# JeffreyXiang/ivid

Hardware: NVIDIA H100
Metric: 128x128 RGBD multiview samples/sec (higher is better)
Workload: dtype fp16 tensor-core operands, fp32 accumulate / residual stream / GroupNorm / softmax / sampler

## Files before the change

ivid_b200/csrc/conv_gemm.cuh:

```cuda
#pragma once
#include <type_traits>

#include "common.cuh"

namespace ivid {

struct ConvGemmParams {
  int N, H, W;
  int TW, TH, TN;
  int tiles_w, tiles_h, tiles_n;
  int n_blocks;
  int seg_chunks[3];
  int seg_taps[3];
  int Cout;
  int ldc;
  int ldr;
  int out_mode;
  const float* bias;
  const float* residual;
  int res_up;
  void* out;
  __half* out16;
  double* stats;
  float acc_scale;
};

struct ConvMaps {
  CUtensorMap a[3];
  CUtensorMap b;
};
struct ConvMaps8 : ConvMaps {
  CUtensorMap b8;
};

template <int BN>
struct ConvGemmCfg {
  static constexpr int BM = 128;
  static constexpr int BK = 64;
  static constexpr int A_BYTES = BM * BK * 2;
  static constexpr int B_BYTES = ((BN * BK * 2 + 1023) / 1024) * 1024;
  static constexpr int STAGE_BYTES = A_BYTES + B_BYTES;
  static constexpr int STAGES = BN == 128 ? 3 : 4;
  static constexpr int BAR_BYTES = 128;
  static constexpr int STAT_BYTES = 8 * 2 * BN * 4;
  static constexpr int SMEM_BYTES = STAGES * STAGE_BYTES + BAR_BYTES + STAT_BYTES + 1024;
  static constexpr int CONSUMER_THREADS = 256;
  static constexpr int THREADS = CONSUMER_THREADS + 32;
};

struct ConvKCursor {
  int seg = 0, t = 0, ch = 0, base = 0;
};

template <int BN, bool A8 = false>
__global__ void __launch_bounds__(ConvGemmCfg<BN>::THREADS, 2)
conv_gemm_kernel(const __grid_constant__ std::conditional_t<A8, ConvMaps8, ConvMaps> maps, const __grid_constant__ ConvGemmParams p) {
  using Cfg = ConvGemmCfg<BN>;
  constexpr int STAGES = Cfg::STAGES;
  extern __shared__ uint8_t smem_raw[];
  uint8_t* smem = smem_raw + ((1024u - (smem_u32(smem_raw) & 1023u)) & 1023u);
  uint64_t* full_bar = reinterpret_cast<uint64_t*>(smem + STAGES * Cfg::STAGE_BYTES);
  uint64_t* empty_bar = full_bar + STAGES;
  float* stat_smem = reinterpret_cast<float*>(smem + STAGES * Cfg::STAGE_BYTES + Cfg::BAR_BYTES);

  const int tid = threadIdx.x;
  const int warp = tid >> 5, lane = tid & 31;
  const int wg = warp >> 2;

  if (tid == 0) {
    for (int s = 0; s < STAGES; ++s) {
      mbar_init(&full_bar[s], 1);
      mbar_init(&empty_bar[s], 8u);
    }
    fence_barrier_init();
  }
  __syncthreads();

  int nunits = 0;
  for (int sg = 0; sg < 3; ++sg) nunits += p.seg_chunks[sg] * p.seg_taps[sg];
  const int nunits8 = A8 ? p.seg_chunks[0] * p.seg_taps[0] : 0;

  const int mt = static_cast<int>(blockIdx.x) / p.n_blocks, nb = static_cast<int>(blockIdx.x) % p.n_blocks;
  const int colbase = nb * BN;
  const int tiles_per_img = p.tiles_w * p.tiles_h;
  const int tn = mt / tiles_per_img;
  const int rem = mt - tn * tiles_per_img;
  const int th = rem / p.tiles_w;
  const int tw = rem - th * p.tiles_w;
  const int n0 = tn * p.TN, h0 = th * p.TH, w0 = tw * p.TW;

  if (warp == Cfg::CONSUMER_THREADS / 32) {
    if (lane == 0) {
      tma_prefetch_desc(&maps.a[0]);
      tma_prefetch_desc(&maps.b);
      if constexpr (A8) tma_prefetch_desc(&maps.b8);
      ConvKCursor c;
      while (p.seg_chunks[c.seg] == 0) ++c.seg;
#pragma unroll 1
      for (int u = 0; u < nunits; ++u) {
        const uint32_t g = static_cast<uint32_t>(u);
        const int s = static_cast<int>(g % STAGES);
        if (g >= STAGES) mbar_wait(&empty_bar[s], ((g / STAGES) - 1) & 1);
        const int taps = p.seg_taps[c.seg], chunks = p.seg_chunks[c.seg];
        uint8_t* sa = smem + s * Cfg::STAGE_BYTES;
        uint8_t* sb = sa + Cfg::A_BYTES;
        const int dy = (taps == 9) ? (c.t / 3 - 1) : 0;
        const int dx = (taps == 9) ? (c.t % 3 - 1) : 0;
        mbar_arrive_expect_tx(&full_bar[s], Cfg::A_BYTES + BN * Cfg::BK * 2);
        bool e4m3 = false;
        if constexpr (A8) {
          if (c.seg == 0) {
            tma_load_4d(&maps.a[0], &full_bar[s], sa, c.ch * 128, w0 + dx, h0 + dy, n0);
            tma_load_2d(&maps.b8, &full_bar[s], sb, (c.t * chunks + c.ch) * 128, colbase);
            e4m3 = true;
          }
        }
        if (!e4m3) {
          const int kcol = c.base + (c.t * chunks + c.ch) * 64;
          tma_load_4d(&maps.a[c.seg], &full_bar[s], sa, c.ch * 64, w0 + dx, h0 + dy, n0);
          tma_load_2d(&maps.b, &full_bar[s], sb, kcol, colbase);
        }
        if (++c.ch == chunks) {
          c.ch = 0;
          if (++c.t == taps) { c.t = 0; if (!A8 || c.seg != 0) c.base += taps * chunks * 64; ++c.seg; }
        }
        while (c.seg < 3 && p.seg_chunks[c.seg] == 0) ++c.seg;
      }
    }
    return;
  }

  float acc[BN / 2];
#pragma unroll
  for (int i = 0; i < BN / 2; ++i) acc[i] = 0.f;

#pragma unroll 1
  for (int u = 0; u < nunits; ++u) {
    const uint32_t g = static_cast<uint32_t>(u);
    const int s = static_cast<int>(g % STAGES);
    mbar_wait(&full_bar[s], (g / STAGES) & 1);
    const uint32_t sa = smem_u32(smem + s * Cfg::STAGE_BYTES);
    const uint32_t sb = sa + Cfg::A_BYTES;
    wgmma_fence();
    const uint64_t da = make_smem_desc_sw128(sa + wg * 64 * 128, 1024, 16);
    const uint64_t db = make_smem_desc_sw128(sb, 1024, 16);
    if (A8 && u < nunits8) {
#pragma unroll
      for (int k = 0; k < 4; ++k) wgmma_ss_e4m3<BN>(acc, da + 2 * k, db + 2 * k, (u | k) != 0 ? 1u : 0u);
    } else {
#pragma unroll
      for (int k = 0; k < 4; ++k) wgmma_ss<BN>(acc, da + 2 * k, db + 2 * k, (u | k) != 0 ? 1u : 0u);
    }
    wgmma_commit();
    wgmma_wait<1>();
    if (u > 0 && lane == 0) mbar_arrive(&empty_bar[(g - 1) % STAGES]);
  }
  wgmma_wait<0>();
  reg_fence(acc);
  if (lane == 0) mbar_arrive(&empty_bar[static_cast<uint32_t>(nunits - 1) % STAGES]);

  const int wr = warp & 3;
  const int quad = lane & 3;
  uint32_t pix[2], rpix[2];
  bool ok[2];
#pragma unroll
  for (int i = 0; i < 2; ++i) {
    const int row = wg * 64 + wr * 16 + (lane >> 2) + 8 * i;
    const int n = n0 + row / (p.TW * p.TH), h = h0 + (row / p.TW) % p.TH, x = w0 + row % p.TW;
    ok[i] = n < p.N;
    pix[i] = (static_cast<uint32_t>(n) * p.H + h) * p.W + x;
    rpix[i] = p.res_up ? (static_cast<uint32_t>(n) * (p.H >> 1) + (h >> 1)) * (p.W >> 1) + (x >> 1) : pix[i];
  }
  const bool do_stats = p.stats != nullptr;
#pragma unroll
  for (int j = 0; j < BN / 8; ++j) {
    const int c = colbase + 8 * j + 2 * quad;
    float s0 = 0.f, s1 = 0.f, q0 = 0.f, q1 = 0.f;
    if (c < p.Cout) {
      const float2 b = make_float2(__ldg(p.bias + c), __ldg(p.bias + c + 1));
#pragma unroll
      for (int i = 0; i < 2; ++i) {
        if (!ok[i]) continue;
        float v0, v1;
        if (A8) {
          v0 = fmaf(acc[4 * j + 2 * i], p.acc_scale, b.x); v1 = fmaf(acc[4 * j + 2 * i + 1], p.acc_scale, b.y);
        } else {
          v0 = acc[4 * j + 2 * i] + b.x; v1 = acc[4 * j + 2 * i + 1] + b.y;
        }
        if (p.out_mode == 2) {
          const uint32_t hw = static_cast<uint32_t>(p.H) * p.W, n = pix[i] / hw;
          float* o = reinterpret_cast<float*>(p.out) + (static_cast<size_t>(n) * p.Cout + c) * hw + (pix[i] - n * hw);
          o[0] = v0;
          if (c + 1 < p.Cout) o[hw] = v1;
          continue;
        }
        if (p.residual != nullptr) {
          const float2 r = __ldg(reinterpret_cast<const float2*>(p.residual + static_cast<size_t>(rpix[i]) * p.ldr + c));
          v0 += r.x; v1 += r.y;
        }
        if (p.out_mode == 0) {
          *reinterpret_cast<float2*>(reinterpret_cast<float*>(p.out) + static_cast<size_t>(pix[i]) * p.ldc + c) = make_float2(v0, v1);
          if (p.out16 != nullptr) *reinterpret_cast<uint32_t*>(p.out16 + static_cast<size_t>(pix[i]) * p.ldc + c) = pack_h2(v0, v1);
        } else {
          const __half2 hv = __floats2half2_rn(v0, v1);
          *reinterpret_cast<__half2*>(reinterpret_cast<__half*>(p.out) + static_cast<size_t>(pix[i]) * p.ldc + c) = hv;
          const float2 r = __half22float2(hv);
          v0 = r.x; v1 = r.y;
        }
        s0 += v0; s1 += v1;
        q0 = fmaf(v0, v0, q0); q1 = fmaf(v1, v1, q1);
      }
    }
    if (do_stats) {
#pragma unroll
      for (int off = 4; off < 32; off <<= 1) {
        s0 += __shfl_xor_sync(0xffffffffu, s0, off);
        s1 += __shfl_xor_sync(0xffffffffu, s1, off);
        q0 += __shfl_xor_sync(0xffffffffu, q0, off);
        q1 += __shfl_xor_sync(0xffffffffu, q1, off);
      }
      if (lane < 4) {
        float* st = stat_smem + warp * 2 * BN + 8 * j + 2 * quad;
        st[0] = s0; st[1] = s1; st[BN] = q0; st[BN + 1] = q1;
      }
    }
  }
  if (do_stats) {
    asm volatile("bar.sync 1, %0;\n" ::"n"(Cfg::CONSUMER_THREADS) : "memory");
    const int rows_per_n = p.TW * p.TH;
    const int n_tile = (128 + rows_per_n - 1) / rows_per_n;
    for (int e = tid; e < n_tile * BN; e += Cfg::CONSUMER_THREADS) {
      const int sn = e / BN, c = e - sn * BN;
      const int n = n0 + sn, col = colbase + c;
      if (n >= p.N || col >= p.Cout) continue;
      float ssum = 0.f, qsum = 0.f;
      for (int w8 = 0; w8 < 8; ++w8) {
        if ((w8 * 16) / rows_per_n != sn) continue;
        ssum += stat_smem[w8 * 2 * BN + c];
        qsum += stat_smem[w8 * 2 * BN + BN + c];
      }
      double* st = p.stats + (static_cast<size_t>(n) * p.Cout + col) * 2;
      atomicAdd(st, static_cast<double>(ssum));
      atomicAdd(st + 1, static_cast<double>(qsum));
    }
  }
}

}
```

ivid_b200/csrc/ops.cu:

```cuda
#include "ops.h"

#include <algorithm>
#include <cmath>
#include <mutex>

#include "attention.cuh"
#include "attention_hd.cuh"
#include "conv_gemm.cuh"
#include "elementwise.cuh"
#include "embed.cuh"

namespace ivid {

struct ConvLaunch {
  ConvMaps8 maps;
  ConvGemmParams p;
  int BN;
  bool a8;
  int grid;
};

int conv_pad_cout(int cout) {
  if (cout >= 64) return ((cout + 63) / 64) * 64;
  return ((cout + 15) / 16) * 16;
}
static int pow2_divisor(int v, int cap) {
  int t = 1;
  while (t * 2 <= cap && v % (t * 2) == 0) t *= 2;
  return t;
}
void conv_tile(int H, int W, int* TW, int* TH, int* TN) {
  IVID_REQUIRE(H > 0 && W > 0, "conv: spatial size must be positive");
  *TW = pow2_divisor(W, 16);
  *TH = pow2_divisor(H, 128 / *TW);
  *TN = 128 / (*TW * *TH);
}
bool conv_can_fuse_stats(int H, int W) {
  int TW, TH, TN;
  conv_tile(H, W, &TW, &TH, &TN);
  return TW * TH >= 32;
}
int conv_pick_bn(int cout_pad) {
  if (cout_pad % 128 == 0) return 128;
  if (cout_pad % 64 == 0) return 64;
  if (cout_pad % 16 == 0 && cout_pad <= 48) return 16;
  throw Error(kErrInvalidArgument, "conv: unsupported padded Cout " + std::to_string(cout_pad));
}

bool conv_can_res_up(int W, int cout) { return W >= 16 && cout % 8 == 0; }
bool conv_can_out16(int cout) { return cout % 8 == 0; }
int conv_pad_k(int c) { return ((c + 63) / 64) * 64; }
int conv_pad_k8(int c) { return ((c + 127) / 128) * 128; }
int conv_seg_cols(int taps, int c) { return taps * conv_pad_k(c); }

ConvPack conv_pack(const float* w, const float* b, int cout, int cin, int ksz, int pitch, const float* w2, const float* b2,
                   int cin2, int cin2a, bool e4m3) {
  ConvPack pk;
  const int taps = ksz * ksz;
  pk.cout_pad = conv_pad_cout(cout);
  float scale = 1.f;
  if (e4m3) {
    IVID_REQUIRE(pitch == conv_pad_k(cin), "internal: an e4m3 segment 0 is an ordinary 3x3 or 1x1 conv");
    float mx = 0.f;
    for (size_t i = 0; i < static_cast<size_t>(cout) * cin * taps; ++i) mx = std::max(mx, std::fabs(w[i]));
    const int e = fp8_weight_exponent(mx);
    const float kMinNormal16 = std::ldexp(1.0f, -14);
    if (cin % 16 != 0) pk.refused = "its input channels are not a multiple of 16";
    else if (e < -100 || e > 100) pk.refused = "its weight exponent is outside [-100, 100]";
    for (size_t i = 0; pk.refused == nullptr && i < static_cast<size_t>(cout) * cin2; ++i) {
      const float v = std::fabs(w2[i]), sv = v * std::ldexp(1.0f, e);
      if (sv > 65504.f) pk.refused = "its skip weights times 2^e overflow fp16";
      else if (v >= kMinNormal16 && sv < kMinNormal16) pk.refused = "its skip weights times 2^e become fp16 subnormals";
    }
    pk.e4m3 = pk.refused == nullptr;
    if (pk.e4m3) { pk.e = e; scale = std::ldexp(1.0f, e); }
  }
  const int s0 = cin2a > 0 ? cin2a : cin2, s1 = cin2 - s0;
  const int k0 = pk.e4m3 ? 0 : conv_seg_cols(1, taps * pitch);
  pk.K = k0 + conv_seg_cols(1, s0) + conv_seg_cols(1, s1);
  pk.w16.assign(static_cast<size_t>(pk.cout_pad) * pk.K, __float2half_rn(0.f));
  const int cp8 = conv_pad_k8(cin), K8 = pk.e4m3 ? taps * cp8 : 0;
  pk.w8.assign(static_cast<size_t>(pk.cout_pad) * K8, 0);
  for (int co = 0; co < cout; ++co) {
    __half* row = pk.w16.data() + static_cast<size_t>(co) * pk.K;
    for (int tap = 0; tap < taps; ++tap)
      for (int ci = 0; ci < cin; ++ci) {
        const float v = w[(static_cast<size_t>(co) * cin + ci) * taps + tap];
        if (pk.e4m3) pk.w8[static_cast<size_t>(co) * K8 + tap * cp8 + ci] = fp8_e4m3_from_float(v * scale);
        else row[tap * pitch + ci] = __float2half_rn(v);
      }
    for (int ci = 0; ci < cin2; ++ci)
      row[k0 + (ci < s0 ? ci : conv_pad_k(s0) + ci - s0)] = __float2half_rn(w2[static_cast<size_t>(co) * cin2 + ci] * scale);
  }
  pk.bias.assign(pk.cout_pad, 0.f);
  for (int i = 0; i < cout; ++i) {
    if (b != nullptr) pk.bias[i] = b[i];
    if (b2 != nullptr) pk.bias[i] += b2[i];
  }
  return pk;
}

ConvLaunch* conv_launch_create(const ConvDesc& d) {
  IVID_REQUIRE(d.C0 > 0 && d.C0 % 8 == 0, "conv: segment-0 channels must be a positive multiple of 8");
  IVID_REQUIRE(d.C1 % 8 == 0, "conv: segment-1 channels must be a multiple of 8");
  IVID_REQUIRE(d.taps0 == 9 || d.taps0 == 1, "conv: only 3x3 (pad 1) and 1x1 kernels are on this path");
  IVID_REQUIRE(d.taps1 == 9 || d.taps1 == 1, "conv: only 3x3 (pad 1) and 1x1 kernels are on this path");
  IVID_REQUIRE(d.C2 % 8 == 0 && (d.taps2 == 9 || d.taps2 == 1), "conv: segment 2 must be a multiple of 8 channels, 3x3 or 1x1");
  IVID_REQUIRE(d.N > 0 && static_cast<int64_t>(d.N) * d.H * d.W < (int64_t{1} << 31),
               "conv: N*H*W must be below 2^31 (32-bit pixel indices in the epilogue)");
  const bool a8 = d.weight8 != nullptr;
  IVID_REQUIRE(!a8 || d.C0 % 16 == 0, "conv: an e4m3 segment 0 needs a multiple of 16 channels (16-byte TMA rows)");
  auto* l = new ConvLaunch();
  l->a8 = a8;
  ConvGemmParams& p = l->p;
  p.N = d.N; p.H = d.H; p.W = d.W;
  conv_tile(d.H, d.W, &p.TW, &p.TH, &p.TN);
  p.tiles_w = d.W / p.TW;
  p.tiles_h = d.H / p.TH;
  p.tiles_n = (d.N + p.TN - 1) / p.TN;
  l->BN = conv_pick_bn(d.cout_pad);
  p.n_blocks = d.cout_pad / l->BN;
  p.seg_chunks[0] = a8 ? conv_pad_k8(d.C0) / 128 : conv_pad_k(d.C0) / 64; p.seg_taps[0] = d.taps0;
  p.acc_scale = d.acc_scale;
  p.seg_chunks[1] = conv_pad_k(d.C1) / 64; p.seg_taps[1] = d.C1 > 0 ? d.taps1 : 0;
  p.seg_chunks[2] = conv_pad_k(d.C2) / 64; p.seg_taps[2] = d.C2 > 0 ? d.taps2 : 0;
  p.Cout = d.cout; p.ldc = d.ldc; p.ldr = d.ldr; p.out_mode = d.out_mode;
  p.bias = d.bias; p.residual = d.residual; p.out = d.out;
  p.stats = (d.stats != nullptr && conv_can_fuse_stats(d.H, d.W) && d.out_mode != 2) ? d.stats : nullptr;
  IVID_REQUIRE(d.stats == nullptr || p.stats != nullptr, "conv: fused statistics need >= 32 pixels per sample per warp");
  IVID_REQUIRE(d.out_mode == 2 || (d.cout % 8 == 0 && d.ldc % 8 == 0), "conv: NHWC output needs Cout % 8 == 0");
  IVID_REQUIRE(d.residual == nullptr || (d.out_mode != 2 && d.ldr % 2 == 0), "conv: residual needs an NHWC output and an even row pitch");
  p.res_up = 0;
  if (d.residual != nullptr && d.residual_up) {
    IVID_REQUIRE(conv_can_res_up(d.W, d.cout) && d.H % 2 == 0, "conv: upsampled residual needs W >= 16 and Cout % 8 == 0");
    p.res_up = 1;
  }
  p.out16 = nullptr;
  if (d.out16 != nullptr) {
    IVID_REQUIRE(d.out_mode == 0 && conv_can_out16(d.cout), "conv: fp16 output copy needs an fp32 NHWC output and Cout % 8 == 0");
    p.out16 = static_cast<__half*>(d.out16);
  }
  const int Ktot = (a8 ? 0 : conv_seg_cols(d.taps0, d.C0)) + conv_seg_cols(d.taps1, d.C1) + conv_seg_cols(d.taps2, d.C2);
  ConvMaps8& M = l->maps;
  M.a[0] = a8 ? make_act_map(d.act0, d.N, d.H, d.W, d.C0, p.TW, p.TH, p.TN, CU_TENSOR_MAP_DATA_TYPE_UINT8)
              : make_act_map(d.act0, d.N, d.H, d.W, d.C0, p.TW, p.TH, p.TN);
  M.a[1] = d.C1 > 0 ? make_act_map(d.act1, d.N, d.H, d.W, d.C1, p.TW, p.TH, p.TN) : M.a[0];
  M.a[2] = d.C2 > 0 ? make_act_map(d.act2, d.N, d.H, d.W, d.C2, p.TW, p.TH, p.TN) : M.a[0];
  if (a8) {
    M.b8 = make_weight_map(d.weight8, d.cout_pad, d.taps0 * conv_pad_k8(d.C0), l->BN, CU_TENSOR_MAP_DATA_TYPE_UINT8);
    M.b = Ktot > 0 ? make_weight_map(d.weight, d.cout_pad, Ktot, l->BN) : M.b8;
  } else {
    M.b = make_weight_map(d.weight, d.cout_pad, Ktot, l->BN);
  }
  l->grid = p.tiles_w * p.tiles_h * p.tiles_n * p.n_blocks;
  return l;
}
void conv_launch_destroy(ConvLaunch* l) { delete l; }
int conv_launch_bn(const ConvLaunch* l) { return l->BN; }
bool conv_launch_a8(const ConvLaunch* l) { return l->a8; }

template <int BN, bool A8>
static void run_conv(const ConvLaunch* l, cudaStream_t s) {
  using Cfg = ConvGemmCfg<BN>;
  static std::once_flag once;
  std::call_once(once, [] {
    IVID_CHECK_CUDA(cudaFuncSetAttribute(conv_gemm_kernel<BN, A8>, cudaFuncAttributeMaxDynamicSharedMemorySize, Cfg::SMEM_BYTES));
  });
  if constexpr (A8) conv_gemm_kernel<BN, true><<<l->grid, Cfg::THREADS, Cfg::SMEM_BYTES, s>>>(l->maps, l->p);
  else conv_gemm_kernel<BN, false><<<l->grid, Cfg::THREADS, Cfg::SMEM_BYTES, s>>>(static_cast<const ConvMaps&>(l->maps), l->p);
  IVID_CHECK_CUDA(cudaGetLastError());
}
void conv_launch_run_out(const ConvLaunch* l, void* out, cudaStream_t s) {
  ConvLaunch tmp = *l;
  tmp.p.out = out;
  conv_launch_run(&tmp, s);
}
void conv_launch_run(const ConvLaunch* l, cudaStream_t s) {
  if (l->a8) {
    switch (l->BN) {
      case 128: run_conv<128, true>(l, s); break;
      case 64: run_conv<64, true>(l, s); break;
      default: run_conv<16, true>(l, s); break;
    }
    return;
  }
  switch (l->BN) {
    case 128: run_conv<128, false>(l, s); break;
    case 64: run_conv<64, false>(l, s); break;
    default: run_conv<16, false>(l, s); break;
  }
}

struct AttnLaunch {
  CUtensorMap mapQ, mapKV;
  AttnParams p;
  AttnHdParams hp;
  int head_ch = 64;
  int nv = 0;
  bool qres = false;
  int smem = 0;
  int grid;
};

AttnLaunch* attn_launch_create(const void* qkv, int N, int T, int C, int head_ch, void* out) {
  if (head_ch <= 0 || head_ch % 64 != 0)
    throw Error(kErrNotImplemented, "attention: head width " + std::to_string(head_ch) + " is not a multiple of 64");
  IVID_REQUIRE(C % head_ch == 0, "attention: channels must be a multiple of the head width " + std::to_string(head_ch));
  IVID_REQUIRE(T >= 1, "attention: sequence length must be positive");
  auto* l = new AttnLaunch();
  l->head_ch = head_ch;
  l->p.N = N; l->p.T = T; l->p.C = C; l->p.heads = C / 64;
  l->p.q_tiles = (T + 127) / 128;
  l->p.out = reinterpret_cast<__half*>(out);
  const uint64_t dims[3] = {static_cast<uint64_t>(3 * C), static_cast<uint64_t>(T), static_cast<uint64_t>(N)};
  const uint64_t str[2] = {static_cast<uint64_t>(3 * C) * 2, static_cast<uint64_t>(T) * 3 * C * 2};
  const uint32_t boxq[3] = {64, 128, 1};
  const uint32_t boxkv[3] = {64, AttnCfg::KV, 1};
  l->mapQ = make_tensor_map(CU_TENSOR_MAP_DATA_TYPE_FLOAT16, 3, const_cast<void*>(qkv), dims, str, boxq,
                            CU_TENSOR_MAP_SWIZZLE_128B);
  l->mapKV = make_tensor_map(CU_TENSOR_MAP_DATA_TYPE_FLOAT16, 3, const_cast<void*>(qkv), dims, str, boxkv,
                             CU_TENSOR_MAP_SWIZZLE_128B);
  l->grid = N * l->p.heads * l->p.q_tiles;
  if (head_ch == 64) return l;
  using Cfg = AttnHdCfg;
  const int k = head_ch / 64;
  const int slices = (k + 3) / 4;
  l->nv = (k + slices - 1) / slices;
  l->qres = k <= Cfg::RESIDENT_Q_MAX_CHUNKS;
  AttnHdParams& hp = l->hp;
  hp.N = N; hp.T = T; hp.C = C; hp.d = head_ch; hp.heads = C / head_ch; hp.chunks = k;
  hp.q_tiles = l->p.q_tiles;
  hp.slices = (k + l->nv - 1) / l->nv;
  hp.scale_log2 = static_cast<float>(1.4426950408889634 / std::sqrt(static_cast<double>(head_ch)));
  hp.out = l->p.out;
  const int q_bytes = l->qres ? k * Cfg::QCHUNK_BYTES : 0;
  const int fixed = q_bytes + 1024  + 1024 ;
  const int budget = l->nv == 2 ? Cfg::MAX_SMEM_2CTA : Cfg::MAX_SMEM;
  hp.stages = std::min(Cfg::MAX_STAGES, (budget - fixed) / Cfg::stage_bytes(l->qres));
  IVID_REQUIRE(hp.stages >= 4, "attention: shared-memory ring too shallow");
  l->smem = fixed + hp.stages * Cfg::stage_bytes(l->qres);
  l->grid = N * hp.heads * hp.q_tiles * hp.slices;
  return l;
}
void attn_launch_destroy(AttnLaunch* l) { delete l; }

template <int NV, bool QRES>
static void run_attn_hd(const AttnLaunch* l, cudaStream_t s) {
  static std::once_flag once;
  std::call_once(once, [] {
    IVID_CHECK_CUDA(cudaFuncSetAttribute(attention_hd_kernel<NV, QRES>, cudaFuncAttributeMaxDynamicSharedMemorySize, AttnHdCfg::MAX_SMEM));
  });
  attention_hd_kernel<NV, QRES><<<l->grid, AttnHdCfg::THREADS, l->smem, s>>>(l->mapQ, l->mapKV, l->hp);
  IVID_CHECK_CUDA(cudaGetLastError());
}

void attn_launch_run(const AttnLaunch* l, cudaStream_t s) {
  if (l->head_ch != 64) {
    switch (l->nv * 2 + (l->qres ? 1 : 0)) {
      case 5: run_attn_hd<2, true>(l, s); break;
      case 7: run_attn_hd<3, true>(l, s); break;
      case 9: run_attn_hd<4, true>(l, s); break;
      case 4: run_attn_hd<2, false>(l, s); break;
      case 6: run_attn_hd<3, false>(l, s); break;
      case 8: run_attn_hd<4, false>(l, s); break;
      default: throw Error(kErrState, "internal: attention slice width " + std::to_string(l->nv));
    }
    return;
  }
  static std::once_flag once;
  std::call_once(once, [] {
    IVID_CHECK_CUDA(cudaFuncSetAttribute(attention_kernel, cudaFuncAttributeMaxDynamicSharedMemorySize, AttnCfg::SMEM_BYTES));
  });
  attention_kernel<<<l->grid, AttnCfg::THREADS, AttnCfg::SMEM_BYTES, s>>>(l->mapQ, l->mapKV, l->p);
  IVID_CHECK_CUDA(cudaGetLastError());
}

static int ew_grid(size_t work_items, int block) {
  const size_t blocks = (work_items + block - 1) / block;
  const size_t cap = static_cast<size_t>(sm_count()) * 16;
  return static_cast<int>(std::max<size_t>(1, std::min(blocks, cap)));
}

void launch_gn_stats(const float* x, double* stats, int N, int HW, int C, cudaStream_t s) {
  IVID_REQUIRE(C % 4 == 0, "gn_stats: C % 4");
  dim3 grid((HW + kStatsPixPerBlock - 1) / kStatsPixPerBlock, N);
  gn_stats_kernel<<<grid, 256, 0, s>>>(x, stats, HW, C);
  IVID_CHECK_CUDA(cudaGetLastError());
}

void launch_gn_apply(const GnApplyDesc& d, cudaStream_t s) {
  IVID_REQUIRE(d.C0 % 8 == 0 && d.C1 % 8 == 0, "gn_apply: channel counts must be multiples of 8");
  const int C = d.C0 + d.C1;
  IVID_REQUIRE(d.groups >= 1 && d.groups <= 64 && C % d.groups == 0, "group norm: groups must divide channels (<= 64 groups)");
  IVID_REQUIRE(d.stats0 != nullptr && d.gamma != nullptr && d.beta != nullptr, "gn_apply: statistics / affine parameters missing");
  GnApplyParams p;
  p.x0 = static_cast<const float*>(d.x0); p.x1 = static_cast<const float*>(d.x1); p.C0 = d.C0; p.C1 = d.C1; p.N = d.N; p.H = d.H; p.W = d.W; p.mode = d.mode;
  p.x0h = d.x0_half ? reinterpret_cast<const __half*>(d.x0) : nullptr;
  p.x1h = d.x0_half ? reinterpret_cast<const __half*>(d.x1) : nullptr;
  p.silu = d.silu ? 1 : 0;
  p.stats0 = d.stats0; p.stats1 = d.stats1; p.groups = d.groups; p.inv_count = 1.0 / (static_cast<double>(d.H) * d.W);
  p.eps = d.eps; p.gamma = d.gamma; p.beta = d.beta; p.film = d.film; p.film_ld = d.film_ld; p.film_off = d.film_off;
  p.film_add = d.film_add ? 1 : 0;
  p.out_act = reinterpret_cast<__half*>(d.out_act); p.out_raw16 = reinterpret_cast<__half*>(d.out_raw16);
  p.out_act8 = d.out_e4m3 ? reinterpret_cast<uint8_t*>(d.out_act) : nullptr;
  p.out_raw32 = d.out_raw32;
  p.out_lo = reinterpret_cast<__half*>(d.out_lo);
  IVID_REQUIRE(d.out_lo == nullptr || (d.mode == 0 && d.x0_half && d.out_raw16 == nullptr && d.out_raw32 == nullptr),
               "gn_apply: the split (hi/lo) output exists on the same-resolution fp16-source path only");
  IVID_REQUIRE(!d.out_e4m3 || (d.out_lo == nullptr && C % 16 == 0), "gn_apply: an e4m3 output needs C % 16 == 0 and no split output");
  const int Ho = d.mode == 1 ? d.H * 2 : (d.mode == 2 ? d.H / 2 : d.H);
  const int Wo = d.mode == 1 ? d.W * 2 : (d.mode == 2 ? d.W / 2 : d.W);
  {
    const int blocks_per_n = std::max(1, (sm_count() * 3) / std::max(d.N, 1));
    const int by_wave = (Ho * Wo + blocks_per_n - 1) / blocks_per_n;
    const int small = std::max(1, 1024 / (C / 8));
    p.pix_per_block = std::max(1, std::min(Ho * Wo, std::max(by_wave, small)));
  }
  int pix_space = Ho * Wo;
  if (d.mode == 1) {
    pix_space = d.H * d.W;
    p.pix_per_block = std::max(1, (p.pix_per_block + 3) / 4);
  }
  dim3 grid((pix_space + p.pix_per_block - 1) / p.pix_per_block, d.N);
  const size_t smem = static_cast<size_t>(C) * 8;
  if (p.mode == 0 && p.x0h != nullptr && p.out_raw16 == nullptr && p.out_raw32 == nullptr) {
    const bool hoist = 256 % (C / 8) == 0;
    if (p.out_lo != nullptr) {
      if (hoist) gn_apply_h16_kernel<true, true><<<grid, 256, smem, s>>>(p);
      else gn_apply_h16_kernel<false, true><<<grid, 256, smem, s>>>(p);
    } else if (d.out_e4m3) {
      if (hoist) gn_apply_h16_kernel<true, false, true><<<grid, 256, smem, s>>>(p);
      else gn_apply_h16_kernel<false, false, true><<<grid, 256, smem, s>>>(p);
    } else if (hoist) gn_apply_h16_kernel<true><<<grid, 256, smem, s>>>(p);
    else gn_apply_h16_kernel<false><<<grid, 256, smem, s>>>(p);
  } else if (d.out_e4m3) {
    gn_apply_kernel<true><<<grid, 256, smem, s>>>(p);
  } else {
    gn_apply_kernel<><<<grid, 256, smem, s>>>(p);
  }
  IVID_CHECK_CUDA(cudaGetLastError());
}
void launch_im2col_s2(const void* x16, void* col, int N, int H, int W, int C, cudaStream_t s) {
  IVID_REQUIRE(C % 8 == 0 && H % 2 == 0 && W % 2 == 0, "im2col_s2: C % 8, even spatial size");
  const size_t items = static_cast<size_t>(N) * (H / 2) * (W / 2) * 9 * (C / 8);
  im2col_s2_h16_kernel<<<ew_grid(items, 256), 256, 0, s>>>(reinterpret_cast<const __half*>(x16), reinterpret_cast<__half*>(col), N, H, W, C);
  IVID_CHECK_CUDA(cudaGetLastError());
}
void launch_upsample2x_h16(const void* x16, void* out, int N, int H, int W, int C, cudaStream_t s) {
  IVID_REQUIRE(C % 8 == 0, "upsample2x: C % 8");
  const size_t items = static_cast<size_t>(N) * H * W * 4 * (C / 8);
  upsample2x_h16_kernel<<<ew_grid(items, 256), 256, 0, s>>>(reinterpret_cast<const __half*>(x16), reinterpret_cast<__half*>(out), N, H, W, C);
  IVID_CHECK_CUDA(cudaGetLastError());
}
void launch_resample_f32(const float* x, float* out, void* out16, int N, int H, int W, int C, int mode, cudaStream_t s) {
  IVID_REQUIRE(C % 4 == 0 && (mode == 1 || (H % 2 == 0 && W % 2 == 0)), "resample_f32: C % 4, even spatial size for pooling");
  const size_t items = static_cast<size_t>(N) * (mode == 1 ? 4 * H * W : (H / 2) * (W / 2)) * (C / 4);
  resample_f32_kernel<<<ew_grid(items, 256), 256, 0, s>>>(x, out, reinterpret_cast<__half*>(out16), N, H, W, C, mode);
  IVID_CHECK_CUDA(cudaGetLastError());
}
void launch_pack_input(const float* x, void* out, int N, int Nx, int Cin, int HW, cudaStream_t s) {
  IVID_REQUIRE(Cin >= 1 && Cin <= 16, "pack_input: 1..16 input channels (two-term split inside 64 operand channels)");
  pack_input_kernel<<<ew_grid(static_cast<size_t>(N) * HW, 256), 256, 0, s>>>(x, reinterpret_cast<__half*>(out), N, Nx,
                                                                                 Cin, HW);
  IVID_CHECK_CUDA(cudaGetLastError());
}

void launch_eps_gather(const float* Y, const float* bias, float* eps, int N, int H, int W, int Co, int ldy, cudaStream_t s) {
  IVID_REQUIRE(Co >= 1 && Co <= 7 && 9 * Co <= ldy, "eps_gather: 9*Co tap columns must fit the row pitch");
  IVID_REQUIRE(Co != 4 || ldy % 4 == 0, "eps_gather: row pitch must keep float4 alignment");
  eps_gather_kernel<<<ew_grid(static_cast<size_t>(N) * H * W, 256), 256, 0, s>>>(Y, bias, eps, N, H, W, Co, ldy);
  IVID_CHECK_CUDA(cudaGetLastError());
}

void launch_posenc(const int64_t* t, int Nt, const float* freqs, int half, float* out, int N, cudaStream_t s) {
  posenc_kernel<<<N, 128, 0, s>>>(t, Nt, freqs, half, out, N);
  IVID_CHECK_CUDA(cudaGetLastError());
}

void launch_film_table(const float* emb, const float* Wp, const float* bias, float* x_t, float* out, int N, int K, int O, cudaStream_t s) {
  IVID_REQUIRE(K % 32 == 0 && O % 4 == 0, "film table: K % 32 == 0");
  static std::once_flag once;
  std::call_once(once, [] {
    IVID_CHECK_CUDA(cudaFuncSetAttribute(film_table_kernel, cudaFuncAttributeMaxDynamicSharedMemorySize, FilmCfg::SMEM_BYTES));
  });
  const int nblk = (N + 31) / 32;
  silu_transpose_kernel<<<std::min(256, (nblk * K * 32 + 255) / 256), 256, 0, s>>>(emb, x_t, N, K, 1);
  const int tiles = (O + FilmCfg::TO - 1) / FilmCfg::TO;
  dim3 grid(std::min(tiles, std::max(1, sm_count() / nblk)), nblk);
  film_table_kernel<<<grid, FilmCfg::THREADS, FilmCfg::SMEM_BYTES, s>>>(Wp, x_t, bias, out, N, K, O);
  IVID_CHECK_CUDA(cudaGetLastError());
}

void launch_linear(const float* in, const float* W, const float* bias, float* out, int N, int K, int O, int silu_in,
                   const float* label_emb, const int64_t* classes, int Ncls, cudaStream_t s) {
  if ((K == 256 || K == 512 || K == 1024) && O <= 8192) {
    dim3 grid((O + 7) / 8, (N + 31) / 32);
    const size_t smem = static_cast<size_t>(32) * K * 4;
    static std::once_flag once;
    std::call_once(once, [] {
      IVID_CHECK_CUDA(cudaFuncSetAttribute(linear_warp_kernel<2>, cudaFuncAttributeMaxDynamicSharedMemorySize, 32 * 256 * 4));
      IVID_CHECK_CUDA(cudaFuncSetAttribute(linear_warp_kernel<4>, cudaFuncAttributeMaxDynamicSharedMemorySize, 32 * 512 * 4));
      IVID_CHECK_CUDA(cudaFuncSetAttribute(linear_warp_kernel<8>, cudaFuncAttributeMaxDynamicSharedMemorySize, 32 * 1024 * 4));
    });
    auto go = [&](auto kern) { kern<<<grid, 256, smem, s>>>(in, W, bias, out, N, O, silu_in, label_emb, classes, Ncls); };
    if (K == 256) go(linear_warp_kernel<2>); else if (K == 512) go(linear_warp_kernel<4>); else go(linear_warp_kernel<8>);
    IVID_CHECK_CUDA(cudaGetLastError());
    return;
  }
  if (K % 32 == 0) {
    if (O >= 128 * 64) {
      dim3 grid((O + 127) / 128, (N + 31) / 32);
      linear_tiled_kernel<4><<<grid, 256, 0, s>>>(in, W, bias, out, N, K, O, silu_in, label_emb, classes, Ncls);
    } else {
      dim3 grid((O + 63) / 64, (N + 31) / 32);
      linear_tiled_kernel<2><<<grid, 256, 0, s>>>(in, W, bias, out, N, K, O, silu_in, label_emb, classes, Ncls);
    }
    IVID_CHECK_CUDA(cudaGetLastError());
    return;
  }
  dim3 grid((O + 63) / 64, (N + 31) / 32);
  linear_rows_kernel<<<grid, 256, 0, s>>>(in, W, bias, out, N, K, O, silu_in, label_emb, classes, Ncls);
  IVID_CHECK_CUDA(cudaGetLastError());
}

}
```

Measured before the change: 0.3019.

## Reuse a halo activation slab across the three vertical taps in 3x3 convs

For 3x3 convolutions with suitable tiles, the producer loads one taller activation slab (tile height plus two halo rows) per horizontal offset and channel chunk. The three vertical taps then read it by offsetting the wgmma descriptor by whole rows, instead of issuing three separate A loads. A two-slab ring with its own empty barriers is split from the weight ring. This cuts TMA activation traffic roughly threefold for the main segment, at the cost of more complex barrier and slab-index bookkeeping and different shared-memory sizing.

```diff
diff --git a/ivid_b200/csrc/conv_gemm.cuh b/ivid_b200/csrc/conv_gemm.cuh
--- a/ivid_b200/csrc/conv_gemm.cuh
+++ b/ivid_b200/csrc/conv_gemm.cuh
@@ -33,7 +33,7 @@
   CUtensorMap b8;
 };
 
-template <int BN>
+template <int BN, bool SLAB = false>
 struct ConvGemmCfg {
   static constexpr int BM = 128;
   static constexpr int BK = 64;
@@ -41,9 +41,12 @@
   static constexpr int B_BYTES = ((BN * BK * 2 + 1023) / 1024) * 1024;
   static constexpr int STAGE_BYTES = A_BYTES + B_BYTES;
   static constexpr int STAGES = BN == 128 ? 3 : 4;
+  static constexpr int SLAB_BYTES = 160 * 128;
+  static constexpr int SLABS = 2;
+  static constexpr int RING_BYTES = SLAB ? SLABS * SLAB_BYTES + STAGES * B_BYTES : STAGES * STAGE_BYTES;
   static constexpr int BAR_BYTES = 128;
   static constexpr int STAT_BYTES = 8 * 2 * BN * 4;
-  static constexpr int SMEM_BYTES = STAGES * STAGE_BYTES + BAR_BYTES + STAT_BYTES + 1024;
+  static constexpr int SMEM_BYTES = RING_BYTES + BAR_BYTES + STAT_BYTES + 1024;
   static constexpr int CONSUMER_THREADS = 256;
   static constexpr int THREADS = CONSUMER_THREADS + 32;
 };
@@ -52,16 +55,19 @@
   int seg = 0, t = 0, ch = 0, base = 0;
 };
 
-template <int BN, bool A8 = false>
+template <int BN, bool A8 = false, bool SLAB = false>
 __global__ void __launch_bounds__(ConvGemmCfg<BN>::THREADS, 2)
 conv_gemm_kernel(const __grid_constant__ std::conditional_t<A8, ConvMaps8, ConvMaps> maps, const __grid_constant__ ConvGemmParams p) {
-  using Cfg = ConvGemmCfg<BN>;
+  using Cfg = ConvGemmCfg<BN, SLAB>;
   constexpr int STAGES = Cfg::STAGES;
+  constexpr int SLABS = Cfg::SLABS;
   extern __shared__ uint8_t smem_raw[];
   uint8_t* smem = smem_raw + ((1024u - (smem_u32(smem_raw) & 1023u)) & 1023u);
-  uint64_t* full_bar = reinterpret_cast<uint64_t*>(smem + STAGES * Cfg::STAGE_BYTES);
+  uint64_t* full_bar = reinterpret_cast<uint64_t*>(smem + Cfg::RING_BYTES);
   uint64_t* empty_bar = full_bar + STAGES;
-  float* stat_smem = reinterpret_cast<float*>(smem + STAGES * Cfg::STAGE_BYTES + Cfg::BAR_BYTES);
+  uint64_t* slab_empty = empty_bar + STAGES;
+  float* stat_smem = reinterpret_cast<float*>(smem + Cfg::RING_BYTES + Cfg::BAR_BYTES);
+  uint8_t* wring = smem + SLABS * Cfg::SLAB_BYTES;
 
   const int tid = threadIdx.x;
   const int warp = tid >> 5, lane = tid & 31;
@@ -71,6 +77,9 @@
     for (int s = 0; s < STAGES; ++s) {
       mbar_init(&full_bar[s], 1);
       mbar_init(&empty_bar[s], 8u);
+    }
+    if constexpr (SLAB) {
+      for (int s = 0; s < SLABS; ++s) mbar_init(&slab_empty[s], 8u);
     }
     fence_barrier_init();
   }
@@ -89,7 +98,59 @@
   const int tw = rem - th * p.tiles_w;
   const int n0 = tn * p.TN, h0 = th * p.TH, w0 = tw * p.TW;
 
-  if (warp == Cfg::CONSUMER_THREADS / 32) {
+  if (SLAB && warp == Cfg::CONSUMER_THREADS / 32) {
+    if (lane == 0) {
+      tma_prefetch_desc(&maps.a[0]);
+      tma_prefetch_desc(&maps.b);
+      if constexpr (A8) tma_prefetch_desc(&maps.b8);
+      uint32_t u = 0, a = 0;
+      auto issue = [&](const CUtensorMap* am, int ac, int ax, int ay, uint32_t a_bytes, const CUtensorMap* bm, int kcol) {
+        const int s = static_cast<int>(u % STAGES);
+        if (u >= STAGES) mbar_wait(&empty_bar[s], ((u / STAGES) - 1) & 1);
+        const int q = static_cast<int>(a % SLABS);
+        if (a_bytes != 0 && a >= SLABS) mbar_wait(&slab_empty[q], ((a / SLABS) - 1) & 1);
+        mbar_arrive_expect_tx(&full_bar[s], a_bytes + BN * Cfg::BK * 2);
+        if (a_bytes != 0) {
+          tma_load_4d(am, &full_bar[s], smem + q * Cfg::SLAB_BYTES, ac, ax, ay, n0);
+          ++a;
+        }
+        tma_load_2d(bm, &full_bar[s], wring + s * Cfg::B_BYTES, kcol, colbase);
+        ++u;
+      };
+      const int chunks0 = p.seg_chunks[0];
+      const uint32_t slab_bytes = static_cast<uint32_t>(p.TW * (p.TH + 2) * p.TN) * 128u;
+#pragma unroll 1
+      for (int dx = 0; dx < 3; ++dx) {
+#pragma unroll 1
+        for (int ch = 0; ch < chunks0; ++ch) {
+#pragma unroll 1
+          for (int dy = 0; dy < 3; ++dy) {
+            const int t = dy * 3 + dx;
+            const uint32_t ab = dy == 0 ? slab_bytes : 0u;
+            if constexpr (A8) issue(&maps.a[0], ch * 128, w0 + dx - 1, h0 - 1, ab, &maps.b8, (t * chunks0 + ch) * 128);
+            else issue(&maps.a[0], ch * 64, w0 + dx - 1, h0 - 1, ab, &maps.b, (t * chunks0 + ch) * 64);
+          }
+        }
+      }
+      int base = A8 ? 0 : 9 * chunks0 * 64;
+#pragma unroll 1
+      for (int sg = 1; sg < 3; ++sg) {
+        const int taps = p.seg_taps[sg], chunks = p.seg_chunks[sg];
+        if (chunks == 0) continue;
+#pragma unroll 1
+        for (int t = 0; t < taps; ++t) {
+          const int dy = (taps == 9) ? (t / 3 - 1) : 0;
+          const int dx = (taps == 9) ? (t % 3 - 1) : 0;
+#pragma unroll 1
+          for (int ch = 0; ch < chunks; ++ch)
+            issue(&maps.a[sg], ch * 64, w0 + dx, h0 + dy, Cfg::A_BYTES, &maps.b, base + (t * chunks + ch) * 64);
+        }
+        base += taps * chunks * 64;
+      }
+    }
+    return;
+  }
+  if (!SLAB && warp == Cfg::CONSUMER_THREADS / 32) {
     if (lane == 0) {
       tma_prefetch_desc(&maps.a[0]);
       tma_prefetch_desc(&maps.b);
@@ -134,15 +195,31 @@
 #pragma unroll
   for (int i = 0; i < BN / 2; ++i) acc[i] = 0.f;
 
+  const int nslab = SLAB ? 9 * p.seg_chunks[0] : 0;
+  const uint32_t slab_row = SLAB ? static_cast<uint32_t>(p.TW) * 128u : 0u;
+  const uint32_t slab_wg = SLAB ? static_cast<uint32_t>((wg * 64) / (p.TW * p.TH) * (p.TH + 2)) * slab_row +
+                                      static_cast<uint32_t>((wg * 64) % (p.TW * p.TH)) * 128u
+                                : 0u;
 #pragma unroll 1
   for (int u = 0; u < nunits; ++u) {
     const uint32_t g = static_cast<uint32_t>(u);
     const int s = static_cast<int>(g % STAGES);
     mbar_wait(&full_bar[s], (g / STAGES) & 1);
-    const uint32_t sa = smem_u32(smem + s * Cfg::STAGE_BYTES);
-    const uint32_t sb = sa + Cfg::A_BYTES;
+    uint32_t sa, sb;
+    if constexpr (SLAB) {
+      sb = smem_u32(wring + s * Cfg::B_BYTES);
+      if (u < nslab) {
+        const int a = u / 3;
+        sa = smem_u32(smem + (a % SLABS) * Cfg::SLAB_BYTES) + slab_wg + static_cast<uint32_t>(u - 3 * a) * slab_row;
+      } else {
+        sa = smem_u32(smem + ((u - 2 * nslab / 3) % SLABS) * Cfg::SLAB_BYTES) + wg * 64 * 128;
+      }
+    } else {
+      sa = smem_u32(smem + s * Cfg::STAGE_BYTES);
+      sb = sa + Cfg::A_BYTES;
+    }
     wgmma_fence();
-    const uint64_t da = make_smem_desc_sw128(sa + wg * 64 * 128, 1024, 16);
+    const uint64_t da = make_smem_desc_sw128(SLAB ? sa : sa + wg * 64 * 128, 1024, 16);
     const uint64_t db = make_smem_desc_sw128(sb, 1024, 16);
     if (A8 && u < nunits8) {
 #pragma unroll
@@ -153,7 +230,14 @@
     }
     wgmma_commit();
     wgmma_wait<1>();
-    if (u > 0 && lane == 0) mbar_arrive(&empty_bar[(g - 1) % STAGES]);
+    if (u > 0 && lane == 0) {
+      mbar_arrive(&empty_bar[(g - 1) % STAGES]);
+      if constexpr (SLAB) {
+        const int v = u - 1;
+        if (v >= nslab) mbar_arrive(&slab_empty[(v - 2 * nslab / 3) % SLABS]);
+        else if (v % 3 == 2) mbar_arrive(&slab_empty[(v / 3) % SLABS]);
+      }
+    }
   }
   wgmma_wait<0>();
   reg_fence(acc);
diff --git a/ivid_b200/csrc/ops.cu b/ivid_b200/csrc/ops.cu
--- a/ivid_b200/csrc/ops.cu
+++ b/ivid_b200/csrc/ops.cu
@@ -17,6 +17,7 @@
   ConvGemmParams p;
   int BN;
   bool a8;
+  bool slab;
   int grid;
 };
 
@@ -141,9 +142,14 @@
     p.out16 = static_cast<__half*>(d.out16);
   }
   const int Ktot = (a8 ? 0 : conv_seg_cols(d.taps0, d.C0)) + conv_seg_cols(d.taps1, d.C1) + conv_seg_cols(d.taps2, d.C2);
+  const int grid = p.tiles_w * p.tiles_h * p.tiles_n * p.n_blocks;
+  l->slab = d.taps0 == 9 && p.TW % 8 == 0 && p.TN == 1 && p.tiles_w * p.tiles_h >= 8;
+  const int box_h0 = l->slab ? p.TH + 2 : p.TH;
+  constexpr int kSlabBytes = ConvGemmCfg<128, true>::SLAB_BYTES;
+  IVID_REQUIRE(!l->slab || p.TW * box_h0 * p.TN * 128 <= kSlabBytes, "internal: conv slab too large");
   ConvMaps8& M = l->maps;
-  M.a[0] = a8 ? make_act_map(d.act0, d.N, d.H, d.W, d.C0, p.TW, p.TH, p.TN, CU_TENSOR_MAP_DATA_TYPE_UINT8)
-              : make_act_map(d.act0, d.N, d.H, d.W, d.C0, p.TW, p.TH, p.TN);
+  M.a[0] = a8 ? make_act_map(d.act0, d.N, d.H, d.W, d.C0, p.TW, box_h0, p.TN, CU_TENSOR_MAP_DATA_TYPE_UINT8)
+              : make_act_map(d.act0, d.N, d.H, d.W, d.C0, p.TW, box_h0, p.TN);
   M.a[1] = d.C1 > 0 ? make_act_map(d.act1, d.N, d.H, d.W, d.C1, p.TW, p.TH, p.TN) : M.a[0];
   M.a[2] = d.C2 > 0 ? make_act_map(d.act2, d.N, d.H, d.W, d.C2, p.TW, p.TH, p.TN) : M.a[0];
   if (a8) {
@@ -152,23 +158,31 @@
   } else {
     M.b = make_weight_map(d.weight, d.cout_pad, Ktot, l->BN);
   }
-  l->grid = p.tiles_w * p.tiles_h * p.tiles_n * p.n_blocks;
+  l->grid = grid;
   return l;
 }
 void conv_launch_destroy(ConvLaunch* l) { delete l; }
 int conv_launch_bn(const ConvLaunch* l) { return l->BN; }
 bool conv_launch_a8(const ConvLaunch* l) { return l->a8; }
 
-template <int BN, bool A8>
+template <int BN, bool A8, bool SLAB>
 static void run_conv(const ConvLaunch* l, cudaStream_t s) {
-  using Cfg = ConvGemmCfg<BN>;
+  using Cfg = ConvGemmCfg<BN, SLAB>;
   static std::once_flag once;
   std::call_once(once, [] {
-    IVID_CHECK_CUDA(cudaFuncSetAttribute(conv_gemm_kernel<BN, A8>, cudaFuncAttributeMaxDynamicSharedMemorySize, Cfg::SMEM_BYTES));
+    IVID_CHECK_CUDA(cudaFuncSetAttribute(conv_gemm_kernel<BN, A8, SLAB>, cudaFuncAttributeMaxDynamicSharedMemorySize, Cfg::SMEM_BYTES));
   });
-  if constexpr (A8) conv_gemm_kernel<BN, true><<<l->grid, Cfg::THREADS, Cfg::SMEM_BYTES, s>>>(l->maps, l->p);
-  else conv_gemm_kernel<BN, false><<<l->grid, Cfg::THREADS, Cfg::SMEM_BYTES, s>>>(static_cast<const ConvMaps&>(l->maps), l->p);
-  IVID_CHECK_CUDA(cudaGetLastError());
+  if constexpr (A8) conv_gemm_kernel<BN, true, SLAB><<<l->grid, Cfg::THREADS, Cfg::SMEM_BYTES, s>>>(l->maps, l->p);
+  else conv_gemm_kernel<BN, false, SLAB><<<l->grid, Cfg::THREADS, Cfg::SMEM_BYTES, s>>>(static_cast<const ConvMaps&>(l->maps), l->p);
+  IVID_CHECK_CUDA(cudaGetLastError());
+}
+template <bool A8, bool SLAB>
+static void run_conv_bn(const ConvLaunch* l, cudaStream_t s) {
+  switch (l->BN) {
+    case 128: run_conv<128, A8, SLAB>(l, s); break;
+    case 64: run_conv<64, A8, SLAB>(l, s); break;
+    default: run_conv<16, A8, SLAB>(l, s); break;
+  }
 }
 void conv_launch_run_out(const ConvLaunch* l, void* out, cudaStream_t s) {
   ConvLaunch tmp = *l;
@@ -177,17 +191,11 @@
 }
 void conv_launch_run(const ConvLaunch* l, cudaStream_t s) {
   if (l->a8) {
-    switch (l->BN) {
-      case 128: run_conv<128, true>(l, s); break;
-      case 64: run_conv<64, true>(l, s); break;
-      default: run_conv<16, true>(l, s); break;
-    }
-    return;
-  }
-  switch (l->BN) {
-    case 128: run_conv<128, false>(l, s); break;
-    case 64: run_conv<64, false>(l, s); break;
-    default: run_conv<16, false>(l, s); break;
+    if (l->slab) run_conv_bn<true, true>(l, s);
+    else run_conv_bn<true, false>(l, s);
+  } else {
+    if (l->slab) run_conv_bn<false, true>(l, s);
+    else run_conv_bn<false, false>(l, s);
   }
 }
 
```

Measured after the change: 0.3056, median of 6. 1.2% higher.
